# AIM-Harvard/pyradiomics

Hardware: AMD Instinct MI355X
Metric: Mvoxels/s for GLCM+GLRLM build, 512^3 vol @32 bins (higher is better)
Workload: dtype u8 levels / u32 counts / f64 out; 1 GPU; GLCM+GLRLM matrix build, 512^3 int32+uint8 volume resident in HBM, 32 grey levels, full mask, 13 angles, uniform levels; one volume per GPU (batch sharding, no collective); size=512, levels=32, dist=uniform, deferred_mode=pipeline

## Files before the change

pyradiomics_amd/csrc/kernels_sweep.h:

```cpp
#pragma once
#include "prad_runtime.h"

namespace prad {

typedef unsigned int u32;
typedef unsigned long long u64;

__global__ void __launch_bounds__(256) pack_levels_kernel(const int *__restrict__ image,
                                                          const uint8_t *__restrict__ mask, long long n, int NX,
                                                          int pitch, int padw, int Ng,
                                                          uint8_t *__restrict__ levels, int *__restrict__ flags,
                                                          int vec_ok, int shift, uint8_t *__restrict__ rowzero = nullptr) {
  const long long tid = (long long)blockIdx.x * blockDim.x + threadIdx.x;
  const long long nthreads = (long long)gridDim.x * blockDim.x;
  const bool linear = (padw == 0 && pitch == NX);
  int bad = 0;
  long long done = 0;
  if (vec_ok) {
    const long long n16 = n >> 4;
    const int upr = NX >> 4;
    const int4 *im4 = reinterpret_cast<const int4 *>(image);
    const uint4 *mk4 = reinterpret_cast<const uint4 *>(mask);
    for (long long t = tid; t < n16; t += nthreads) {
      const uint4 m = mk4[t];
// ... 682 lines not shown
    int y = r / Nx, x = r - y * Nx;
    const int pz = z - dz, py = y - dy, px = x - dx;
    if ((unsigned)pz < (unsigned)Nz && (unsigned)py < (unsigned)Ny && (unsigned)px < (unsigned)Nx) continue;
    int cnt = 0;
    while ((unsigned)z < (unsigned)Nz && (unsigned)y < (unsigned)Ny && (unsigned)x < (unsigned)Nx) {
      cnt += L[((long long)z * Ny + y) * pitch + x] != 0;
      if (cnt > 1) {
        multi[a] = 1;
        return;
      }
      z += dz; y += dy; x += dx;
    }
  }
}

__global__ void finalize_glcm_kernel(const u32 *__restrict__ acc, const u32 *__restrict__ glrlm_acc, int Ng, int Nr,
                                     int Na, int diag_from_runs, double *__restrict__ out) {
  const long long idx = (long long)blockIdx.x * blockDim.x + threadIdx.x;
  const long long total = (long long)Ng * Ng * Na;
  if (idx >= total) return;
  const int a = (int)(idx % Na);
  const long long ij = idx / Na;
  const int i = (int)(ij / Ng), j = (int)(ij - (long long)i * Ng);
  if (diag_from_runs && i == j) return;
  out[idx] = (double)acc[(size_t)a * Ng * Ng + ij];
}

__global__ void __launch_bounds__(256) finalize_glcm_diag_kernel(const u32 *__restrict__ glcm_acc, u32 *glrlm_acc, int Ng, int Nr,
                                                                 int Na, int nb1, double *__restrict__ glcm_out,
                                                                 int *__restrict__ multi, int restore_from = -1) {
  if ((int)blockIdx.x < nb1) {
    const long long idx = (long long)blockIdx.x * blockDim.x + threadIdx.x;
    const long long total = (long long)Ng * Ng * Na;
    if (idx >= total) return;
    const int a = (int)(idx % Na);
    const long long ij = idx / Na;
    const int i = (int)(ij / Ng), j = (int)(ij - (long long)i * Ng);
    if (i == j) return;
    glcm_out[idx] = (double)glcm_acc[(size_t)a * Ng * Ng + ij];
    return;
  }
  const int pair = ((int)blockIdx.x - nb1) * 4 + (int)(threadIdx.x >> 6), lane = threadIdx.x & 63;
  if (pair >= Ng * Na) return;
  const int i = pair % Ng, a = pair / Ng;
  u32 *row = glrlm_acc + ((size_t)a * Ng + i) * Nr;
  unsigned long long pairs = 0, longer = 0;
  int found = 0;
  for (int r = lane; r < Nr; r += 64) {
    const u32 v = row[r];
    pairs += (unsigned long long)r * v;
    if (r > 0) longer += v;
    found |= (r > 0 && v != 0);
  }
  const u32 *grow = glcm_acc + ((size_t)a * Ng + i) * Ng;
  for (int j = lane; j < Ng; j += 64) found |= (grow[j] != 0);
  for (int o = 32; o > 0; o >>= 1) pairs += __shfl_xor(pairs, o);
  if (lane == 0) glcm_out[((size_t)i * Ng + i) * Na + a] = (double)pairs;
  if (__ballot(found) != 0 && lane == 0) multi[a] = 1;
  if (restore_from >= 0 && a != restore_from) {
    const u32 *xrow = glrlm_acc + ((size_t)restore_from * Ng + i) * Nr;
    unsigned long long nvox = 0;
    for (int r = lane; r < Nr; r += 64) nvox += (unsigned long long)(r + 1) * xrow[r];
    for (int o = 32; o > 0; o >>= 1) {
      nvox += __shfl_xor(nvox, o);
      longer += __shfl_xor(longer, o);
    }
    if (lane == 0) row[0] = (u32)(nvox - (pairs + longer));
  }
}

__global__ void finalize_glrlm_kernel(const u32 *__restrict__ acc, const int *__restrict__ multi, int Ng, int Nr,
                                      int Na, double *__restrict__ out, const int *__restrict__ flags = nullptr,
                                      int *__restrict__ sticky = nullptr) {
  if (sticky && blockIdx.x == 0 && threadIdx.x == 0 && (flags[0] || flags[2])) sticky[0] = 1;
  const long long idx = (long long)blockIdx.x * blockDim.x + threadIdx.x;
  const long long total = (long long)Ng * Nr * Na;
  if (idx >= total) return;
  const int a = (int)(idx % Na);
  const long long gr = idx / Na;
  const int r = (int)(gr % Nr);
  out[idx] = (r == 0 && !multi[a]) ? 0.0 : (double)acc[(size_t)a * Ng * Nr + gr];
}

}
```

pyradiomics_amd/csrc/prad_api.hip:

```cpp
#include "prad_runtime.h"
#include "kernels_generic.h"
#include "kernels_pairs.h"
#include "kernels_sweep.h"
#include "kernels_sweepfw.h"
#include "kernels_sweepfw2.h"
#include "kernels_neigh.h"
#include "kernels_glszm.h"
#include "kernels_voxel.h"
#include "kernels_voxslide.h"
#include "kernels_mcc.h"
#include "kernels_voxtex.h"
#include "kernels_binning.h"

#include <algorithm>
#include <atomic>
#include <chrono>
#include <cmath>
#include <condition_variable>
#include <cstdlib>
#include <deque>
#include <limits>
#include <mutex>
#include <thread>

using namespace prad;

namespace {

const char *kVersion = "pyradiomics_amd 0.1.0 (gfx950)";

int angle_count(const int *size, const int *distances, int Nd, int Ndist, int bidirectional, int f2d) {
  long long total = 0;
  for (int k = 0; k < Ndist; k++) {
    const int dist = distances[k];
    if (dist < 1) return 0;
    long long shell_outer = 1, shell_inner = 1;
    for (int d = 0; d < Nd; d++) {
      if (d == f2d) continue;
      if (dist < size[d]) {
        shell_outer *= 2LL * dist + 1;
        shell_inner *= 2LL * dist - 1;
      } else {
        const long long reach = 2LL * (size[d] - 1) + 1;
        shell_outer *= reach;
        shell_inner *= reach;
      }
    }
    total += shell_outer - shell_inner;
  }
  if (!bidirectional) total /= 2;
  return (int)total;
}

int angle_build(const int *size, const int *distances, int Nd, int Ndist, int f2d, int Na, int *angles) {
  int maxd = 0;
  for (int k = 0; k < Ndist; k++) {
    if (distances[k] < 1) return 1;
    maxd = std::max(maxd, distances[k]);
  }
  std::vector<int> off(Nd, maxd);
  int got = 0;
  long long guard = 1;
  for (int d = 0; d < Nd; d++) guard *= (2LL * maxd + 1);
  for (long long it = 0; it < guard && got < Na; it++) {
    int norm = 0;
    bool legal = true;
    for (int d = 0; d < Nd && legal; d++) {
      const int o = off[d];
      if ((d == f2d && o != 0) || o >= size[d] || o <= -size[d]) legal = false;
      norm = std::max(norm, std::abs(o));
    }
    if (legal && norm >= 1) {
      for (int k = 0; k < Ndist; k++)
        if (distances[k] == norm) {
          std::copy(off.begin(), off.end(), angles + (size_t)got * Nd);
          got++;
          break;
        }
    }
    for (int d = Nd - 1; d >= 0; d--) {
      if (off[d] > -maxd) { off[d]--; break; }
      off[d] = maxd;
    }
  }
  return got == Na ? 0 : 1;
}

struct Call {
  Context *c;
  hipStream_t s;
  Geo g;
  VoxMode vm;
  const int32_t *image;
  const uint8_t *mask;
  const int *angles_h;
  int *angles_d;
  int Na;
  int *flags_d;
  int *flags_h;
};

int setup_call(Call &k, const int32_t *image, const uint8_t *mask, const int *size, int Nd, const int *angles,
               int Na, int Nvox, const int *voxels_dev, int kernelRadius, int force2Ddim, hipStream_t s,
               bool zero_flags = true) {
  Context &c = ctx();
  k.c = &c;
  k.s = s;
  if (!image || !mask) return fail(PRAD_E_ARG, "image/mask is NULL");
  if (!angles || Na < 1) return fail(PRAD_E_ARG, "angles is NULL or Na < 1");
  PRAD_TRY(make_geo(size, Nd, &k.g));
  if (Nvox < 1) return fail(PRAD_E_ARG, "Nvox=%d < 1", Nvox);
  k.vm.nvox = Nvox;
  k.vm.voxels = voxels_dev;
  k.vm.radius = kernelRadius;
  k.vm.f2d = force2Ddim;
  if (voxels_dev) {
    if (kernelRadius <= 0) return fail(PRAD_E_ARG, "Expecting kernelRadius > 0");
    long long b = 1;
    for (int d = 0; d < Nd; d++)
      if (d != force2Ddim) b *= std::min<long long>(2LL * kernelRadius + 1, k.g.size[d]);
    k.vm.boxmax = b;
  } else {
    if (Nvox != 1) return fail(PRAD_E_ARG, "Nvox=%d without a voxel list", Nvox);
    k.vm.boxmax = k.g.n;
  }
  k.image = image;
  k.mask = mask;
  k.angles_h = angles;
  k.Na = Na;
  {
    int *prev = nullptr;
    auto it = c.bufs.find(c.key("angles"));
    if (it != c.bufs.end()) prev = (int *)it->second.p;
    PRAD_TRY(c.get<int>("angles", (size_t)Na * Nd, &k.angles_d));
    std::vector<int> &cached = c.angle_cache();
    const bool same = prev == k.angles_d && cached.size() == (size_t)Na * Nd &&
                      std::equal(cached.begin(), cached.end(), angles);
    if (!same) {
      PRAD_HIP(hipMemcpyAsync(k.angles_d, angles, sizeof(int) * Na * Nd, hipMemcpyHostToDevice, s));
      PRAD_HIP(hipStreamSynchronize(s));
      cached.assign(angles, angles + (size_t)Na * Nd);
    }
  }
  PRAD_TRY(c.get<int>("flags", 4, &k.flags_d));
  if (zero_flags) PRAD_HIP(hipMemsetAsync(k.flags_d, 0, sizeof(int) * 4, s));
  void *fh = nullptr;
  PRAD_TRY(c.get_pinned("flags_h", sizeof(int) * 4, &fh));
  k.flags_h = (int *)fh;
  return PRAD_OK;
}

int read_flags(Call &k) {
  PRAD_HIP(hipMemcpyAsync(k.flags_h, k.flags_d, sizeof(int) * 4, hipMemcpyDeviceToHost, k.s));
  PRAD_HIP(hipStreamSynchronize(k.s));
  return PRAD_OK;
}

inline unsigned blocks_for(long long threads, int bs = 256) { return (unsigned)((threads + bs - 1) / bs); }

int check_grid(long long threads, const char *what) {
  if ((threads + 255) / 256 > 2147483647LL)
    return fail(PRAD_E_UNSUPPORTED, "%s: %lld work items exceed the launch grid; split the voxel batch", what, threads);
  return PRAD_OK;
}

int generic_glcm(Call &k, int Ng, double *out) {
  const size_t per = (size_t)Ng * Ng * k.Na;
  PRAD_HIP(hipMemsetAsync(out, 0, sizeof(double) * per * k.vm.nvox, k.s));
  const long long threads = (long long)k.vm.nvox * k.vm.boxmax;
  PRAD_TRY(check_grid(threads, "GLCM"));
  Timed t(*k.c, "generic", k.s);
  hipLaunchKernelGGL(gen_glcm_kernel, dim3(blocks_for(threads)), dim3(256), 0, k.s, k.g, k.vm, k.image, k.mask,
                     k.angles_d, k.Na, Ng, out, k.flags_d + 1);
  return check_launch("gen_glcm_kernel");
}

int generic_glrlm(Call &k, int Ng, int Nr, double *out) {
  const size_t per = (size_t)Ng * Nr * k.Na;
  PRAD_HIP(hipMemsetAsync(out, 0, sizeof(double) * per * k.vm.nvox, k.s));
  int *multi = nullptr;
  PRAD_TRY(k.c->get<int>("multi", (size_t)k.vm.nvox * k.Na, &multi));
  PRAD_HIP(hipMemsetAsync(multi, 0, sizeof(int) * k.vm.nvox * k.Na, k.s));
  const long long threads = (long long)k.vm.nvox * k.vm.boxmax * k.Na;
  PRAD_TRY(check_grid(threads, "GLRLM"));
  Timed t(*k.c, "generic", k.s);
  hipLaunchKernelGGL(gen_glrlm_kernel, dim3(blocks_for(threads)), dim3(256), 0, k.s, k.g, k.vm, k.image, k.mask,
                     k.angles_d, k.Na, Ng, Nr, out, multi, k.flags_d + 1);
  PRAD_TRY(check_launch("gen_glrlm_kernel"));
  const long long pthreads = (long long)k.vm.nvox * Ng * k.Na;
  hipLaunchKernelGGL(glrlm_prune_kernel, dim3(blocks_for(pthreads)), dim3(256), 0, k.s, out, multi, k.vm.nvox, Ng,
                     Nr, k.Na);
  return check_launch("glrlm_prune_kernel");
}

int generic_gldm(Call &k, int Ng, int alpha, double *out) {
  const size_t per = (size_t)Ng * (2 * (size_t)k.Na + 1);
  PRAD_HIP(hipMemsetAsync(out, 0, sizeof(double) * per * k.vm.nvox, k.s));
  const long long threads = (long long)k.vm.nvox * k.vm.boxmax;
  PRAD_TRY(check_grid(threads, "GLDM"));
  Timed t(*k.c, "generic", k.s);
  hipLaunchKernelGGL(gen_gldm_kernel, dim3(blocks_for(threads)), dim3(256), 0, k.s, k.g, k.vm, k.image, k.mask,
                     k.angles_d, k.Na, Ng, alpha, out, k.flags_d + 1);
  return check_launch("gen_gldm_kernel");
}

int generic_ngtdm(Call &k, int Ng, double *out) {
  Timed t(*k.c, "generic", k.s);
  if (k.vm.voxels) {
    hipLaunchKernelGGL(gen_ngtdm_voxel_kernel, dim3(blocks_for(k.vm.nvox, 64)), dim3(64), 0, k.s, k.g, k.vm,
                       k.image, k.mask, k.angles_d, k.Na, Ng, out, k.flags_d + 1);
    return check_launch("gen_ngtdm_voxel_kernel");
  }
  unsigned long long *acc = nullptr;
  const size_t nacc = (size_t)Ng * (k.Na + 1);
  PRAD_TRY(k.c->get<unsigned long long>("ngtdm_acc", nacc, &acc));
  PRAD_HIP(hipMemsetAsync(acc, 0, sizeof(unsigned long long) * nacc, k.s));
  PRAD_TRY(check_grid(k.g.n, "NGTDM"));
  hipLaunchKernelGGL(gen_ngtdm_segment_kernel, dim3(blocks_for(k.g.n)), dim3(256), 0, k.s, k.g, k.vm, k.image,
                     k.mask, k.angles_d, k.Na, Ng, acc, k.flags_d + 1);
  PRAD_TRY(check_launch("gen_ngtdm_segment_kernel"));
  hipLaunchKernelGGL(ngtdm_finalize_kernel, dim3(blocks_for(Ng, 64)), dim3(64), 0, k.s, acc, Ng, k.Na, out);
  return check_launch("ngtdm_finalize_kernel");
}

struct SweepPlan {
  bool ok = false;
  int Nz = 1, Ny = 1, Nx = 1;
  SweepSet lines;
// ... 377 lines not shown
                   int *work, int *flags_d) {
  if (pj.n16 > 0) return launch_fw2_khsp<LNG, K, HASPAD, SKIP1, true>(k, p, pj, levels16, Ng, Nr, glcm_acc, glrlm_acc, work, flags_d);
  return launch_fw2_khsp<LNG, K, HASPAD, SKIP1, false>(k, p, pj, levels16, Ng, Nr, glcm_acc, glrlm_acc, work, flags_d);
}
template <bool LNG, int K>
int launch_fw2_k(Call &k, const SweepPlan &p, const PackJob &pj, const uint8_t *levels16, int Ng, int Nr, u32 *glcm_acc, u32 *glrlm_acc,
                 int *multi, int *flags_d) {
  int *work = multi + 2 * PRAD_MAX_SWEEP + PRAD_FW_WORK_STRIDE;
  if (p.Nx != 64 * K)
    return p.skip1 ? launch_fw2_khs<LNG, K, true, true>(k, p, pj, levels16, Ng, Nr, glcm_acc, glrlm_acc, work, flags_d)
                   : launch_fw2_khs<LNG, K, true, false>(k, p, pj, levels16, Ng, Nr, glcm_acc, glrlm_acc, work, flags_d);
  return p.skip1 ? launch_fw2_khs<LNG, K, false, true>(k, p, pj, levels16, Ng, Nr, glcm_acc, glrlm_acc, work, flags_d)
                 : launch_fw2_khs<LNG, K, false, false>(k, p, pj, levels16, Ng, Nr, glcm_acc, glrlm_acc, work, flags_d);
}
int launch_fw2(Call &k, const SweepPlan &p, const PackJob &pj, const uint8_t *levels16, int Ng, int Nr, u32 *glcm_acc, u32 *glrlm_acc,
               int *multi, int *flags_d) {
  if (p.LONGfw2) return p.fwK == 4 ? launch_fw2_k<true, 4>(k, p, pj, levels16, Ng, Nr, glcm_acc, glrlm_acc, multi, flags_d)
                                 : launch_fw2_k<true, 8>(k, p, pj, levels16, Ng, Nr, glcm_acc, glrlm_acc, multi, flags_d);
  return p.fwK == 4 ? launch_fw2_k<false, 4>(k, p, pj, levels16, Ng, Nr, glcm_acc, glrlm_acc, multi, flags_d)
                    : launch_fw2_k<false, 8>(k, p, pj, levels16, Ng, Nr, glcm_acc, glrlm_acc, multi, flags_d);
}

template <bool LNG>
int launch_fw_rows(Call &k, const SweepPlan &p, const uint8_t *levels, int Ng, int Nr, u32 *glcm_acc, u32 *glrlm_acc, int *flags_d) {
  const long long nrows = (long long)p.Nz * p.Ny, groups = nrows >= 4096 ? ((nrows + 511) / 512) * 8 : (nrows + 63) / 64;
  const int wpb = p.fw_rows_threads / 64;
  const unsigned gx = (unsigned)std::max<long long>(1, std::min<long long>((groups + wpb - 1) / wpb, (long long)cu_count()));
  PRAD_HIP(hipFuncSetAttribute(reinterpret_cast<const void *>(&sweep_fw_rows_kernel<LNG>),
                               hipFuncAttributeMaxDynamicSharedMemorySize, (int)p.lds_fw_rows));
  hipLaunchKernelGGL((sweep_fw_rows_kernel<LNG>), dim3(gx), dim3(p.fw_rows_threads), p.lds_fw_rows, k.s, levels, nrows, p.Nx,
                     p.pitch, p.row_slot, Ng, Nr, p.RSfw_rows, glcm_acc, glrlm_acc, flags_d);
  return check_launch("sweep_fw_rows_kernel");
}

template <bool LNG>
int launch_fw2_rows(Call &k, const SweepPlan &p, const uint8_t *levels16, int Ng, int Nr, u32 *glcm_acc, u32 *glrlm_acc, int *flags_d) {
  const long long nrows = (long long)p.Nz * p.Ny, groups = nrows >= 4096 ? ((nrows + 511) / 512) * 8 : (nrows + 63) / 64;
  const int wpb = p.fw2r_waves;
  const unsigned gx = (unsigned)std::max<long long>(1, std::min<long long>((groups + wpb - 1) / wpb, (long long)cu_count()));
  PRAD_HIP(hipFuncSetAttribute(reinterpret_cast<const void *>(&sweep_fw2_rows_kernel<LNG>),
                               hipFuncAttributeMaxDynamicSharedMemorySize, (int)p.lds_fw2_rows));
  hipLaunchKernelGGL((sweep_fw2_rows_kernel<LNG>), dim3(gx), dim3(64 * wpb), p.lds_fw2_rows, k.s, levels16, nrows, p.Nx, p.pitch16,
                     p.row_slot, Ng, Nr, p.RS2r, p.fw2r_copies, glcm_acc, glrlm_acc, flags_d);
  return check_launch("sweep_fw2_rows_kernel");
}

template <bool G, bool R, bool LNG, bool F>
int launch_rows(Call &k, const SweepPlan &p, const uint8_t *levels, int Ng, int Nr, u32 *glcm_acc, u32 *glrlm_acc,
                int *multi) {
  const long long nrows = (long long)p.Nz * p.Ny;
  const long long groups = (nrows + 63) / 64;
  const int wpb = kRowsThreads / 64;
  const int per_cu = std::max(1, std::min(2048 / kRowsThreads, (int)(160 * 1024 / p.lds_bytes_rows)));
  const unsigned gx = (unsigned)std::max<long long>(1, std::min<long long>((groups + wpb - 1) / wpb, (long long)cu_count() * per_cu));
  PRAD_HIP(hipFuncSetAttribute(reinterpret_cast<const void *>(&sweep_rows_kernel<G, R, LNG, F>),
                               hipFuncAttributeMaxDynamicSharedMemorySize, (int)p.lds_bytes_rows));
  hipLaunchKernelGGL((sweep_rows_kernel<G, R, LNG, F>), dim3(gx), dim3(kRowsThreads), p.lds_bytes_rows, k.s, levels,
                     nrows, p.Nx, p.pitch, p.row_slot, Ng, Nr, p.RSr, glcm_acc, glrlm_acc, multi, k.flags_d);
  return check_launch("sweep_rows_kernel");
}

__global__ void __launch_bounds__(256) zero3_kernel(u32 *__restrict__ a, size_t na, u32 *__restrict__ b, size_t nb,
                                                    u32 *__restrict__ c3, size_t nc) {
  const size_t t = (size_t)blockIdx.x * blockDim.x + threadIdx.x, nt = (size_t)gridDim.x * blockDim.x;
  uint4 *a4 = reinterpret_cast<uint4 *>(a);
  for (size_t i = t; i < na / 4; i += nt) a4[i] = make_uint4(0, 0, 0, 0);
  for (size_t i = (na & ~(size_t)3) + t; i < na; i += nt) a[i] = 0;
  for (size_t i = t; i < nb; i += nt) b[i] = 0;
  for (size_t i = t; i < nc; i += nt) c3[i] = 0;
}

struct VolState {
  bool valid = false;
  SweepPlan p;
  int Ng = 0, Nr = 0, Na = 0;
  double *glcm = nullptr, *glrlm = nullptr;
  uint8_t *levels = nullptr, *rowzero = nullptr;
  uint8_t *levels16 = nullptr;
  u32 *acc = nullptr, *glcm_acc = nullptr, *glrlm_acc = nullptr;
  int *multi = nullptr;
  int *flags_d = nullptr;
  bool packed_inline = false;
  int lane = -1;
};

bool fin_side() {
  static const bool on = getenv("PRAD_FINALIZE_STREAM") != nullptr && atoi(getenv("PRAD_FINALIZE_STREAM")) != 0;
  return on;
}
int fin_wait_for_lane(hipStream_t s, int lane);

int vol_prepare(Call &k, const SweepPlan &p, int Ng, int Nr, double *glcm, double *glrlm, VolState &v) {
  Context &c = *k.c;
  if (fin_side() && c.lane >= 0) PRAD_TRY(fin_wait_for_lane(k.s, c.lane));
  v.lane = c.lane;
  v.valid = true;
  v.p = p;
  v.Ng = Ng;
  v.Nr = Nr;
  v.Na = k.Na;
  v.glcm = glcm;
  v.glrlm = glrlm;
  v.flags_d = k.flags_d;
  const long long nrows = (long long)p.Nz * p.Ny;
  v.levels = nullptr;
  if (!(p.fw2 && p.fw2_rows && p.lines.count > 0 && p.row_slot >= 0) || getenv("PRAD_FW2_KEEP8")) {
    PRAD_TRY(c.get<uint8_t>("levels", (size_t)nrows * p.pitch + 1024, &v.levels));
    v.levels += 512;
  }
  v.levels16 = nullptr;
  if (p.fw2) {
    PRAD_TRY(c.get<uint8_t>("levels16", (size_t)nrows * p.pitch16 + 4096, &v.levels16));
    v.levels16 += 2048;
  }
  const size_t nglcm = glcm ? (size_t)k.Na * Ng * Ng : 0, nglrlm = glrlm ? (size_t)k.Na * Ng * Nr : 0;
  const size_t nctl = 2 * PRAD_MAX_SWEEP + (size_t)PRAD_FW_WORK_STRIDE * (PRAD_FW_DOMAINS * PRAD_MAX_SWEEP + 1);
  PRAD_TRY(c.get<u32>("sweep_acc", nglcm + nglrlm + nctl, &v.acc));
  v.glcm_acc = v.acc;
  v.glrlm_acc = v.acc + nglcm;
  v.multi = (int *)(v.acc + nglcm + nglrlm);
  v.rowzero = nullptr;
  if (p.fw) PRAD_TRY(c.get<uint8_t>("rowzero", (size_t)nrows + 64, &v.rowzero));
  const size_t acc_w = nglcm + nglrlm + nctl, rz_w = v.rowzero ? ((size_t)nrows + 3) / 4 : 0;
  const size_t total_w = acc_w + rz_w + 4;
  const unsigned gx = (unsigned)std::max<size_t>(1, std::min<size_t>((total_w / 4 + 255) / 256, 1024));
  hipLaunchKernelGGL(zero3_kernel, dim3(gx), dim3(256), 0, k.s, v.acc, acc_w, reinterpret_cast<u32 *>(v.rowzero), rz_w,
                     reinterpret_cast<u32 *>(v.flags_d), (size_t)4);
  return check_launch("zero3_kernel");
}

bool pipeline_volume(const SweepPlan &p, bool glcm, bool glrlm) {
  if (!(p.ok && p.lines.count > 0 && glcm && glrlm)) return false;
  return (p.fw && p.fused) || (p.fw2 && !getenv("PRAD_FW2_LANES"));
}
bool pack_inline_ok(const Call &k, const VolState &v) {
  if (!(v.glcm && v.glrlm && v.p.pitch == v.p.Nx && v.p.padw == 0 && (k.g.n % 16) == 0 &&
        ((((uintptr_t)k.image) | ((uintptr_t)k.mask) | ((uintptr_t)v.levels)) & 15) == 0))
    return false;
  if (k.g.n >= (1LL << 31)) return false;
  if (v.p.fw2) return v.levels16 && v.p.pitch16 == 2 * v.p.Nx && (((uintptr_t)v.levels16) & 15) == 0;
  return v.p.fw && v.p.fused;
}

PackJob make_pack_job(const Call &k, const VolState &v, const VolState *host) {
  PackJob j;
  memset(&j, 0, sizeof(j));
  j.image = k.image;
  j.mask = k.mask;
  j.levels = v.levels;
  j.levels16 = v.p.fw2 ? v.levels16 : nullptr;
  j.rowzero = v.rowzero;
  j.flags = v.flags_d;
  j.n16 = k.g.n / 16;
  j.NX = v.p.Nx;
  j.Ng = v.Ng;
  double groups = 0, waves = 16.0;
  if (host) {
    for (int i = 0; i < host->p.fwset.count; i++) groups += (double)host->p.fwset.d[i].NM * host->p.fwset.d[i].NU / PRAD_FW_U;
    waves = 16.0 * std::max(1, host->p.fw_blocks);
  }
  const double units = (double)j.n16 / 64.0;
  const double slack = v.p.fw2 ? 1.05 : 0.92;
  j.every = (int)std::max(1.0, std::min(64.0, std::floor(slack * groups / std::max(1.0, units))));
  (void)waves;
  if (const char *e = getenv("PRAD_PACK_EVERY")) j.every = std::max(1, atoi(e));
  return j;
}

int vol_pack_standalone(Call &k, VolState &v) {
  Context &c = *k.c;
  const SweepPlan &p = v.p;
  Timed t(c, "pack", k.s);
  if (p.fw2) {
    const unsigned gx = (unsigned)std::max<long long>(1, std::min<long long>((k.g.n / 4 + 255) / 256, 8192));
    hipLaunchKernelGGL(pack_levels16_kernel, dim3(gx), dim3(256), 0, k.s, k.image, k.mask, k.g.n, p.Nx, p.pitch16, p.pitch, v.Ng,
                       v.levels16, v.levels, v.flags_d);
    return check_launch("pack_levels16_kernel");
  }
  const int vec_ok = p.vec_rows && ((((uintptr_t)k.image) | ((uintptr_t)k.mask) | ((uintptr_t)v.levels)) & 15) == 0;
  const unsigned gx = (unsigned)std::max<long long>(1, std::min<long long>((k.g.n / 16 + 255) / 256, 4096));
  const int shift = (v.glcm && v.glrlm && p.fused) ? PRAD_FUSED_SHIFT : 0;
  hipLaunchKernelGGL(pack_levels_kernel, dim3(gx), dim3(256), 0, k.s, k.image, k.mask, k.g.n, p.Nx, p.pitch, p.padw,
                     v.Ng, v.levels, v.flags_d, vec_ok, shift, v.rowzero);
  return check_launch("pack_levels_kernel");
}

template <bool G, bool R, bool F>
int launch_sweeps(Call &k, const VolState &v, const PackJob &pj) {
  const SweepPlan &p = v.p;
  if (p.lines.count > 0 && p.fw && G && R && F) {
    static const bool rows_side = getenv("PRAD_ROWS_STREAM") != nullptr;
    if (rows_side && p.row_slot >= 0) {
      static thread_local hipStream_t side = nullptr;
      static thread_local hipEvent_t e0 = nullptr, e1 = nullptr;
      if (!side) {
        int lo = 0, hi = 0;
        PRAD_HIP(hipDeviceGetStreamPriorityRange(&lo, &hi));
        PRAD_HIP(hipStreamCreateWithPriority(&side, hipStreamNonBlocking, getenv("PRAD_ROWS_STREAM_PRIO") ? atoi(getenv("PRAD_ROWS_STREAM_PRIO")) : lo));
        PRAD_HIP(hipEventCreateWithFlags(&e0, hipEventDisableTiming));
        PRAD_HIP(hipEventCreateWithFlags(&e1, hipEventDisableTiming));
      }
      PRAD_HIP(hipEventRecord(e0, k.s));
      PRAD_HIP(hipStreamWaitEvent(side, e0, 0));
      {
        Timed t(*k.c, "sweep", k.s);
        PRAD_TRY(launch_fw(k, p, pj, v.levels, v.rowzero, v.Ng, v.Nr, v.glcm_acc, v.glrlm_acc, v.multi, v.flags_d));
// ... 3 lines not shown
      if (p.RSfw_rows < v.Nr) PRAD_TRY(launch_fw_rows<true>(k2, p, v.levels, v.Ng, v.Nr, v.glcm_acc, v.glrlm_acc, v.flags_d));
      else PRAD_TRY(launch_fw_rows<false>(k2, p, v.levels, v.Ng, v.Nr, v.glcm_acc, v.glrlm_acc, v.flags_d));
      PRAD_HIP(hipEventRecord(e1, side));
      PRAD_HIP(hipStreamWaitEvent(k.s, e1, 0));
      return PRAD_OK;
    }
    {
      Timed t(*k.c, "sweep", k.s);
      PRAD_TRY(launch_fw(k, p, pj, v.levels, v.rowzero, v.Ng, v.Nr, v.glcm_acc, v.glrlm_acc, v.multi, v.flags_d));
    }
    if (p.row_slot >= 0) {
      Timed t(*k.c, "rows", k.s);
      if (p.RSfw_rows < v.Nr) PRAD_TRY(launch_fw_rows<true>(k, p, v.levels, v.Ng, v.Nr, v.glcm_acc, v.glrlm_acc, v.flags_d));
      else PRAD_TRY(launch_fw_rows<false>(k, p, v.levels, v.Ng, v.Nr, v.glcm_acc, v.glrlm_acc, v.flags_d));
    }
    return PRAD_OK;
  }
  if (p.fw2 && G && R && !F && p.lines.count > 0) {
    {
      Timed t(*k.c, "sweep", k.s);
      PRAD_TRY(launch_fw2(k, p, pj, v.levels16, v.Ng, v.Nr, v.glcm_acc, v.glrlm_acc, v.multi, v.flags_d));
    }
    if (p.row_slot >= 0) {
      Timed t(*k.c, "rows", k.s);
      if (p.fw2_rows) {
        if (p.LONGfw2r) PRAD_TRY(launch_fw2_rows<true>(k, p, v.levels16, v.Ng, v.Nr, v.glcm_acc, v.glrlm_acc, v.flags_d));
        else PRAD_TRY(launch_fw2_rows<false>(k, p, v.levels16, v.Ng, v.Nr, v.glcm_acc, v.glrlm_acc, v.flags_d));
      } else if (p.LONGr) {
        PRAD_TRY((launch_rows<G, R, true, F>(k, p, v.levels, v.Ng, v.Nr, v.glcm_acc, v.glrlm_acc, v.multi)));
      } else {
        PRAD_TRY((launch_rows<G, R, false, F>(k, p, v.levels, v.Ng, v.Nr, v.glcm_acc, v.glrlm_acc, v.multi)));
      }
    }
    return PRAD_OK;
  }
  Timed t(*k.c, "sweep", k.s);
  if (p.lines.count > 0) {
    if (R && p.LONG) PRAD_TRY((launch_lines<G, R, true, F>(k, p, v.levels, v.Ng, v.Nr, v.glcm_acc, v.glrlm_acc, v.multi)));
    else PRAD_TRY((launch_lines<G, R, false, F>(k, p, v.levels, v.Ng, v.Nr, v.glcm_acc, v.glrlm_acc, v.multi)));
  }
  if (p.row_slot >= 0) {
    if (R && p.LONGr) PRAD_TRY((launch_rows<G, R, true, F>(k, p, v.levels, v.Ng, v.Nr, v.glcm_acc, v.glrlm_acc, v.multi)));
    else PRAD_TRY((launch_rows<G, R, false, F>(k, p, v.levels, v.Ng, v.Nr, v.glcm_acc, v.glrlm_acc, v.multi)));
  }
  return PRAD_OK;
}

int vol_sweep(Call &k, const VolState &v, const PackJob &pj) {
  if (pj.n16 > 0 && !pipeline_volume(v.p, v.glcm != nullptr, v.glrlm != nullptr))
    return fail(PRAD_E_ARG, "internal: a pack job needs a fixed-window host launch");
  if (pj.n16 > 0 && (pj.levels16 != nullptr) != v.p.fw2)
    return fail(PRAD_E_ARG, "internal: the pack job's layout is not the host launch's");
  if (v.glcm && v.glrlm && v.p.fused) return launch_sweeps<true, true, true>(k, v, pj);
  if (v.glcm && v.glrlm) return launch_sweeps<true, true, false>(k, v, pj);
  if (v.glcm) return launch_sweeps<true, false, false>(k, v, pj);
  return launch_sweeps<false, true, false>(k, v, pj);
}

__global__ void latch_flags_kernel(const int *__restrict__ flags, int *__restrict__ sticky) {
  if (flags[0] || flags[2]) sticky[0] = 1;
}

__global__ void latch_any_flag_kernel(const int *__restrict__ flags, int *__restrict__ sticky) {
  if (flags[0] || flags[1] || flags[2]) sticky[0] = 1;
}
int latch_neigh(Context &c, Call &k) {
  int *sticky = nullptr;
  PRAD_TRY(c.get<int>("deferred_sticky", 16, &sticky));
  hipLaunchKernelGGL(latch_any_flag_kernel, dim3(1), dim3(1), 0, k.s, (const int *)k.flags_d, sticky);
  return check_launch("latch_any_flag_kernel");
}

int vol_finalize(Call &k, const VolState &v, int *sticky) {
  Context &c = *k.c;
  const SweepPlan &p = v.p;
  const int Ng = v.Ng, Nr = v.Nr, Na = v.Na;
  double *glcm = v.glcm, *glrlm = v.glrlm;
  bool latched = false;
  {
    Timed t(c, "finalize", k.s);
    const bool runs_diag = p.fused || p.fw2;
    if (p.fw2 && p.skip1 && p.lines.count > 0 && !(glcm && glrlm && p.row_slot >= 0))
      return fail(PRAD_E_UNSUPPORTED, "sweep plan derives runs of length 1 but the call cannot restore them");
    if (glcm && glrlm && runs_diag) {
      const int nb1 = (int)blocks_for((long long)Ng * Ng * Na), nb2 = (Ng * Na + 3) / 4;
      hipLaunchKernelGGL(finalize_glcm_diag_kernel, dim3(nb1 + nb2), dim3(256), 0, k.s, v.glcm_acc, v.glrlm_acc, Ng, Nr, Na, nb1,
                         glcm, v.multi, (p.fw2 && p.skip1 && p.lines.count > 0) ? p.row_slot : -1);
      PRAD_TRY(check_launch("finalize_glcm_diag_kernel"));
    } else if (glcm) {
      hipLaunchKernelGGL(finalize_glcm_kernel, dim3(blocks_for((long long)Ng * Ng * Na)), dim3(256), 0, k.s,
                         v.glcm_acc, v.glrlm_acc, Ng, Nr, Na, p.fused ? 1 : 0, glcm);
      PRAD_TRY(check_launch("finalize_glcm_kernel"));
    }
    if (glrlm && runs_diag) {
      if (!glcm) {
        hipLaunchKernelGGL(glcm_diag_resolve_kernel, dim3(Ng, Na), dim3(64), 0, k.s, v.glcm_acc, v.glrlm_acc, Ng, Nr, Na,
                           glcm, v.multi);
        PRAD_TRY(check_launch("glcm_diag_resolve_kernel"));
      }
      if (v.levels)
        hipLaunchKernelGGL(multi_check_kernel<uint8_t>, dim3(128, Na), dim3(256), 0, k.s, p.aset, (const uint8_t *)v.levels, p.Nz, p.Ny,
                           p.Nx, p.pitch, v.multi);
      else
        hipLaunchKernelGGL(multi_check_kernel<unsigned short>, dim3(128, Na), dim3(256), 0, k.s, p.aset,
                           reinterpret_cast<const unsigned short *>(v.levels16), p.Nz, p.Ny, p.Nx, p.pitch16 / 2, v.multi);
      PRAD_TRY(check_launch("multi_check_kernel"));
    }
    if (glrlm) {
      hipLaunchKernelGGL(finalize_glrlm_kernel, dim3(blocks_for((long long)Ng * Nr * Na)), dim3(256), 0, k.s,
                         v.glrlm_acc, v.multi, Ng, Nr, Na, glrlm, (const int *)v.flags_d, sticky);
      PRAD_TRY(check_launch("finalize_glrlm_kernel"));
      latched = sticky != nullptr;
    }
  }
  if (sticky && !latched) {
    hipLaunchKernelGGL(latch_flags_kernel, dim3(1), dim3(1), 0, k.s, v.flags_d, sticky);
    PRAD_TRY(check_launch("latch_flags_kernel"));
  }
  return PRAD_OK;
}

int sweep_glcm_glrlm(Call &k, const SweepPlan &p, int Ng, int Nr, double *glcm, double *glrlm, bool *used) {
  Context &c = *k.c;
  VolState v;
  PRAD_TRY(vol_prepare(k, p, Ng, Nr, glcm, glrlm, v));
  PRAD_TRY(vol_pack_standalone(k, v));
  PackJob pj;
  memset(&pj, 0, sizeof(pj));
  PRAD_TRY(vol_sweep(k, v, pj));
  int *sticky = nullptr;
  if (c.deferred) PRAD_TRY(c.get<int>("deferred_sticky", 16, &sticky));
  PRAD_TRY(vol_finalize(k, v, sticky));
  if (c.deferred) {
    *used = true;
    return PRAD_OK;
  }
  PRAD_TRY(read_flags(k));
  *used = (k.flags_h[0] == 0 && k.flags_h[2] == 0);
  return PRAD_OK;
}

struct PipeState {
  VolState pending;
  hipStream_t s = nullptr;
  unsigned long long seq = 0;
  hipEvent_t ev = nullptr;
  int mode = -1;
  hipStream_t fin = nullptr;
  hipEvent_t fin_in = nullptr, fin_all = nullptr, fin_done[4] = {};
  bool fin_used[4] = {};
};
PipeState &pipe_state() {
  static thread_local PipeState p;
  return p;
}
bool pipeline_mode() {
  PipeState &ps = pipe_state();
  if (ps.mode < 0) {
    const char *e = getenv("PRAD_DEFERRED_MODE");
    ps.mode = (e && strcmp(e, "lanes") == 0) ? 0 : 1;
  }
  return ps.mode == 1;
}
int pipeline_sticky(Context &c, int **sticky) { return c.get<int>("deferred_sticky", 16, sticky); }

int pipeline_retire(Context &c, hipStream_t s, const PackJob &pj) {
// ... 136 lines not shown
      RT = PRAD_PAIR_LDS_WORDS / Ng;
      ntile = (Ng + RT - 1) / RT;
    }
    const int npass = ((k.Na + AG - 1) / AG) * ntile;
    const size_t lds = sizeof(u32) * (size_t)AG * RT * Ng;
    PRAD_HIP(hipFuncSetAttribute(reinterpret_cast<const void *>(&pairs_glcm_kernel), hipFuncAttributeMaxDynamicSharedMemorySize, (int)lds));
    long long gbest = 1;
    double ebest = 0;
    for (long long gtry = std::max<long long>(1, 2LL * cus / npass); gtry <= std::max<long long>(1, (4LL * cus + npass - 1) / npass); gtry++) {
      const long long total = gtry * npass, rounds = (total + cus - 1) / cus;
      const double eff = (double)total / (double)(rounds * cus);
      if (eff > ebest + 1e-9) {
        ebest = eff;
        gbest = gtry;
      }
    }
    const unsigned gx = (unsigned)std::max<long long>(1, std::min<long long>((k.g.n / 8 + 1023) / 1024, gbest));
    hipLaunchKernelGGL(pairs_glcm_kernel, dim3(gx, (unsigned)npass), dim3(1024), lds, s, L, dims[0], dims[1], dims[2], A, AG, RT,
                       ntile, Ng, gacc, k.flags_d);
    PRAD_TRY(check_launch("pairs_glcm_kernel"));
    const long long total = (long long)Ng * Ng * k.Na;
    hipLaunchKernelGGL(finalize_glcm_kernel, dim3(blocks_for(total)), dim3(256), 0, s, gacc, (const u32 *)nullptr, Ng, 1, k.Na, 0, glcm);
    PRAD_TRY(check_launch("finalize_glcm_kernel"));
  }
  if (glrlm) {
    Timed t(c, "pairs", s);
    PRAD_HIP(hipMemsetAsync(racc, 0, sizeof(u32) * rwords, s));
    PRAD_HIP(hipMemsetAsync(counts, 0, sizeof(u32) * (size_t)Ng, s));
    PRAD_HIP(hipMemsetAsync(multi, 0, sizeof(int) * PRAD_PAIR_MAXA, s));
    const int use_lds = Ng <= 8192;
    const unsigned gc = (unsigned)std::max<long long>(1, std::min<long long>((k.g.n + 255) / 256, (long long)cus * 8));
    hipLaunchKernelGGL(pairs_level_count_kernel, dim3(gc), dim3(256), use_lds ? sizeof(u32) * (size_t)Ng : 0, s, L, k.g.n, Ng, use_lds,
                       counts, k.flags_d);
    PRAD_TRY(check_launch("pairs_level_count_kernel"));
    const unsigned gx = (unsigned)std::max<long long>(1, std::min<long long>((k.g.n + 255) / 256, std::max(1LL, 16LL * cus / k.Na)));
    hipLaunchKernelGGL(pairs_glrlm_kernel, dim3(gx, (unsigned)k.Na), dim3(256), 0, s, L, dims[0], dims[1], dims[2], A, Ng, Nr, racc, multi,
                       k.flags_d);
    PRAD_TRY(check_launch("pairs_glrlm_kernel"));
    hipLaunchKernelGGL(pairs_multi_check_kernel, dim3(gx, (unsigned)k.Na), dim3(256), 0, s, A, L, dims[0], dims[1], dims[2], multi, k.flags_d);
    PRAD_TRY(check_launch("pairs_multi_check_kernel"));
    hipLaunchKernelGGL(pairs_run1_kernel, dim3((unsigned)((Ng * k.Na + 3) / 4)), dim3(256), 0, s, racc, counts, Ng, Nr, k.Na, k.flags_d);
    PRAD_TRY(check_launch("pairs_run1_kernel"));
    const long long total = (long long)Ng * Nr * k.Na;
    hipLaunchKernelGGL(finalize_glrlm_kernel, dim3(blocks_for(total)), dim3(256), 0, s, racc, multi, Ng, Nr, k.Na, glrlm,
                       (const int *)nullptr, (int *)nullptr);
    PRAD_TRY(check_launch("finalize_glrlm_kernel"));
  }
  PRAD_TRY(read_flags(k));
  *used = k.flags_h[0] == 0;
  if (!*used) {
    PRAD_HIP(hipMemsetAsync(k.flags_d, 0, sizeof(int) * 4, s));
  }
  return PRAD_OK;
}

int texture_pairs_runs(const int32_t *image, const uint8_t *mask, const int *size, int Nd, const int *angles,
                       int Na, int Ng, int Nr, int Nvox, const int *voxels, int kernelRadius, int force2Ddim,
                       double *glcm, double *glrlm, hipStream_t s) {
  if (!glcm && !glrlm) return fail(PRAD_E_ARG, "both outputs are NULL");
  if (Ng < 1 || (glrlm && Nr < 1)) return fail(PRAD_E_ARG, "Ng/Nr must be >= 1");
  Context &c = ctx();
  PRAD_TRY(c.ensure_device());
  struct LaneGuard {
    Context &c;
    ~LaneGuard() { c.lane = -1; }
  } lane_guard{c};
  bool pipe = c.deferred && !voxels && pipeline_mode();
  if (c.deferred && !voxels && !pipe) PRAD_TRY(c.lane_begin(s, &s));
  if (pipe) c.lane = (int)(pipe_state().seq++ % (fin_side() ? 3u : 2u));
  Call k;
  PRAD_TRY(setup_call(k, image, mask, size, Nd, angles, Na, Nvox, voxels, kernelRadius, force2Ddim, s, false));
  SweepPlan p = plan_sweep(k, Ng, Nr, glcm != nullptr, glrlm != nullptr);
  if (pipe && !pipeline_volume(p, glcm != nullptr, glrlm != nullptr)) {
    const hipStream_t user = s;
    PRAD_TRY(pipeline_flush(c));
    pipe = false;
    c.lane = -1;
    PRAD_TRY(c.lane_begin(user, &s));
    if (c.lane >= 0) c.lane += fin_side() ? 3 : 2;
    PRAD_TRY(setup_call(k, image, mask, size, Nd, angles, Na, Nvox, voxels, kernelRadius, force2Ddim, s, false));
    p = plan_sweep(k, Ng, Nr, glcm != nullptr, glrlm != nullptr);
  }
  PRAD_TRY(c.begin_call(s));
  if (!p.ok) PRAD_HIP(hipMemsetAsync(k.flags_d, 0, sizeof(int) * 4, s));
  bool done = false;
  c.last_variant = !p.ok ? "none" : (p.fw2 ? "fw2" : (p.fw && glcm && glrlm ? "fw" : "lines"));
  if (pipe) {
    PRAD_TRY(pipeline_step(k, p, Ng, Nr, glcm, glrlm, &done));
    if (done) c.last_path = "sweep";
  }
  if (!done && p.ok) {
    PRAD_TRY(sweep_glcm_glrlm(k, p, Ng, Nr, glcm, glrlm, &done));
    if (done) c.last_path = "sweep";
  }
  if (!done && !c.deferred) {
    PRAD_TRY(pairs_glcm_glrlm(k, Ng, Nr, glcm, glrlm, &done));
    if (done) {
      c.last_path = "pairs";
      c.last_variant = "pairs";
    }
  }
  if (!done) {
    if (glcm) PRAD_TRY(generic_glcm(k, Ng, glcm));
    if (glrlm) PRAD_TRY(generic_glrlm(k, Ng, Nr, glrlm));
    PRAD_TRY(read_flags(k));
    c.last_path = "generic";
  }
  PRAD_TRY(c.end_call(s));
  if (c.deferred && done) return PRAD_OK;
  PRAD_HIP(hipStreamSynchronize(s));
  return k.flags_h[1] ? PRAD_INDEX_ERROR : PRAD_OK;
}

int pairs_neigh(Call &k, bool ngtdm, int Ng, int alpha, double *out, bool *used, bool box_only = false) {
  *used = false;
  Context &c = *k.c;
  if (k.vm.voxels || k.g.nd > 3 || Ng < 1 || Ng > 65535 || k.g.n >= 0x7fffffffLL || getenv("PRAD_NO_PAIRS")) return PRAD_OK;
  int dims[3] = {1, 1, 1};
  for (int d = 0; d < k.g.nd; d++) dims[3 - k.g.nd + d] = k.g.size[d];
  int rad[3] = {0, 0, 0};
  bool box = ngtdm && !getenv("PRAD_NGTDM_NO_BOX");
  long long cube = 1;
  if (box) {
    for (int a = 0; a < k.Na; a++)
      for (int d = 0; d < k.g.nd; d++) rad[3 - k.g.nd + d] = std::max(rad[3 - k.g.nd + d], std::abs(k.angles_h[a * k.g.nd + d]));
    cube = (long long)(2 * rad[0] + 1) * (2 * rad[1] + 1) * (2 * rad[2] + 1);
    box = cube - 1 == k.Na && cube <= 4096 && cube * Ng < (1LL << 40);
    if (box) {
      std::vector<char> seen((size_t)cube, 0);
      for (int a = 0; box && a < k.Na; a++) {
        long long idx = 0;
        bool zero = true;
        for (int d = 0; d < 3; d++) {
          const int o = d < 3 - k.g.nd ? 0 : k.angles_h[a * k.g.nd + (d - (3 - k.g.nd))];
          zero = zero && o == 0;
          idx = idx * (2 * rad[d] + 1) + (o + rad[d]);
        }
        if (zero || seen[(size_t)idx]) box = false;
        else seen[(size_t)idx] = 1;
      }
    }
  }
  if (box_only && !box) return PRAD_OK;
  if (!box && k.Na > PRAD_PAIR_MAXA) return PRAD_OK;
  PairAngles A;
  memset(&A, 0, sizeof(A));
  A.n = std::min(k.Na, PRAD_PAIR_MAXA);
  for (int a = 0; a < A.n; a++)
    for (int d = 0; d < k.g.nd; d++) {
      const int o = k.angles_h[a * k.g.nd + d];
      if (o < -127 || o > 127) return PRAD_OK;
      A.o[a][3 - k.g.nd + d] = (signed char)o;
    }
  const size_t nacc = (size_t)Ng * (k.Na + 1);
  if (nacc * sizeof(u64) > ((size_t)1 << 30)) return PRAD_OK;
  hipStream_t s = k.s;
  lev16 *L = nullptr;
  u32 *acc32 = nullptr;
  u64 *acc64 = nullptr;
  PRAD_TRY(c.get<lev16>("pairs_levels", (size_t)k.g.n + 8, &L));
  if (ngtdm) PRAD_TRY(c.get<u64>("pairs_ngtdm_acc", nacc, &acc64));
  else PRAD_TRY(c.get<u32>("pairs_gldm_acc", nacc, &acc32));
  PRAD_HIP(hipMemsetAsync(k.flags_d, 0, sizeof(int) * 4, s));
  const int cus = cu_count();
  {
    Timed t(c, "pack", s);
    const unsigned gx = (unsigned)std::max<long long>(1, std::min<long long>((k.g.n + 255) / 256, (long long)cus * 16));
    hipLaunchKernelGGL(pairs_pack_kernel, dim3(gx), dim3(256), 0, s, k.image, k.mask, k.g.n, Ng, L, k.flags_d);
    PRAD_TRY(check_launch("pairs_pack_kernel"));
  }
  {
    Timed t(c, "pairs", s);
    if (ngtdm) PRAD_HIP(hipMemsetAsync(acc64, 0, sizeof(u64) * nacc, s));
    else PRAD_HIP(hipMemsetAsync(acc32, 0, sizeof(u32) * nacc, s));
    const size_t budget = (size_t)PRAD_PAIR_LDS_WORDS * 4;
    int mode = 0;
    size_t lds = 0;
// ... 407 lines not shown
extern "C" {

const char *prad_version(void) { return kVersion; }
const char *prad_last_error(void) { return err_state().msg; }
const char *prad_last_path(void) { return ctx().last_path; }
const char *prad_last_variant(void) { return ctx().last_variant; }
#ifdef PRAD_FW_STAMPS
int prad_debug_fw_stamps(unsigned long long *out, int slot, int nwaves) {
  if (!out || nwaves < 1 || nwaves > 8192 || slot < 0 || slot > 1) return PRAD_E_ARG;
  PRAD_HIP(hipDeviceSynchronize());
  PRAD_HIP(hipMemcpyFromSymbol(out, HIP_SYMBOL(prad::prad_fw_stamps), sizeof(unsigned long long) * prad::FP_COUNT * (size_t)nwaves,
                               sizeof(unsigned long long) * prad::FP_COUNT * 8192 * (size_t)slot));
  return PRAD_OK;
}
#endif

int prad_device_count(void) {
  int n = 0;
  if (hipGetDeviceCount(&n) != hipSuccess) return 0;
  return n;
}

int prad_set_device(int device) {
  int n = prad_device_count();
  if (device < 0 || device >= n) return fail(PRAD_E_ARG, "device %d not in [0,%d)", device, n);
  Context &c = ctx();
  if (c.device != device) {
    if (pipe_state().pending.valid && c.device_set && hipSetDevice(c.device) == hipSuccess) {
      (void)pipeline_flush(c);
      if (pipe_state().s) (void)hipStreamSynchronize(pipe_state().s);
      (void)fin_join(nullptr, true);
    }
    pipe_state().pending.valid = false;
    pipe_state().s = nullptr;
    pipe_state().ev = nullptr;
    pipe_state().fin = nullptr;
    for (int l = 0; l < 4; l++) pipe_state().fin_used[l] = false;
    c.own_stream = nullptr;
    for (int l = 0; l < PRAD_MAX_LANES; l++) {
      if (c.lane_stream[l]) (void)hipStreamSynchronize(c.lane_stream[l]);
      c.lane_stream[l] = nullptr;
      c.lane_in[l] = nullptr;
    }
    c.event_pool.clear();
    c.events_used = 0;
  }
  c.device = device;
  c.device_set = true;
  PRAD_HIP(hipSetDevice(device));
  return PRAD_OK;
}
int prad_get_device(void) { return ctx().device; }

long long prad_workspace_bytes(void) {
  long long total = 0;
  for (const auto &kv : ctx().bufs) total += (long long)kv.second.cap;
  return total;
}
namespace {
void release_image_queues();
}
int prad_release_workspace(void) {
  Context &c = ctx();
  if (pipe_state().pending.valid) {
    (void)pipeline_flush(c);
    if (pipe_state().s) (void)hipStreamSynchronize(pipe_state().s);
    (void)fin_join(nullptr, true);
    pipe_state().pending.valid = false;
  }
  glszm_state().valid = false;
  for (auto &kv : c.bufs) {
    if (kv.second.p) (void)hipFree(kv.second.p);
    kv.second.p = nullptr;
    kv.second.cap = 0;
  }
  (void)hipDeviceSynchronize();
  for (auto &kv : c.pinned) {
    if (kv.second.p) (void)hipHostFree(kv.second.p);
    kv.second.p = nullptr;
    kv.second.cap = 0;
  }
  c.bufs.clear();
  c.pinned.clear();
  if (c.arena) (void)hipHostFree(c.arena);
  c.arena = nullptr;
  c.arena_pos = 0;
  release_image_queues();
  c.angles_cached.clear();
  StageRing &r = stage_ring();
  for (int i = 0; i < kStageRing; i++) {
    r.buf[i] = nullptr;
    r.busy[i] = false;
  }
  return PRAD_OK;
}

int prad_timing_begin(void) {
  Context &c = ctx();
  c.timing_only.clear();
  c.timing_accumulate = true;
  c.all_times.clear();
  c.all_calls.clear();
  c.events_used = 0;
  return PRAD_OK;
}
int prad_timing_begin_only(const char *kernel_family) {
  if (!kernel_family || !*kernel_family) return fail(PRAD_E_ARG, "timing: no kernel family named");
  int rc = prad_timing_begin();
  ctx().timing_only = kernel_family;
  return rc;
}
int prad_timing_count(const char *kernel_family) {
  Context &c = ctx();
  if (!kernel_family) return (int)c.all_calls.size();
  int n = 0;
  for (auto &t : c.all_times) n += t.family == kernel_family;
  return n;
}
int prad_timing_end(void) {
  Context &c = ctx();
  c.timing_only.clear();
  c.timing_accumulate = false;
  c.all_times.clear();
  c.all_calls.clear();
  return PRAD_OK;
}
int prad_timing_calls(void) { return (int)ctx().all_calls.size(); }
double prad_timing_ms(const char *family) {
  Context &c = ctx();
  double total = 0;
  if (!family) {
    for (auto &ab : c.all_calls) {
      float ms = 0;
      if (hipEventSynchronize(ab.second) != hipSuccess || hipEventElapsedTime(&ms, ab.first, ab.second) != hipSuccess) return -1.0;
      total += ms;
    }
    return total;
  }
  for (auto &t : c.all_times) {
    if (t.family != family) continue;
    float ms = 0;
    if (hipEventSynchronize(t.b) != hipSuccess || hipEventElapsedTime(&ms, t.a, t.b) != hipSuccess) return -1.0;
    total += ms;
  }
  return total;
}

int prad_set_deferred(int on) {
  Context &c = ctx();
  if (c.ensure_device() != PRAD_OK) return PRAD_E_HIP;
  if (on && !c.has("deferred_sticky")) {
    int *sticky = nullptr;
    PRAD_TRY(c.get<int>("deferred_sticky", 16, &sticky));
    PRAD_HIP(hipMemset(sticky, 0, sizeof(int) * 16));
  }
  c.deferred = on != 0;
  return PRAD_OK;
}
int prad_set_lanes(int n) {
  Context &c = ctx();
  if (n < 0 || n > PRAD_MAX_LANES) return fail(PRAD_E_ARG, "lanes=%d outside [0, %d]", n, PRAD_MAX_LANES);
  PRAD_TRY(c.lanes_sync());
  c.lanes = n;
  c.lane_seq = 0;
  return PRAD_OK;
}
// ... 673 lines not shown
```

Baseline: 287,200 Mvoxels/s.

## Fuse GLCM/GLRLM finalize, multi-check and accumulator zeroing into one tail kernel

Adds a single finalize_tail_kernel per angle that computes the GLCM diagonal from run counts, restores length-1 runs, performs the multi-run check, writes both f64 outputs and zeroes the accumulators, control words and rowzero for the next call. Host-side state tracks whether the accumulators are already clean, so the next vol_prepare can skip the full zero3 clear or only clear the leftover slice. This removes several small kernel launches and a separate memset pass per volume. The cost is more complex cross-call state that must be invalidated correctly, and a fallback multi-check scan inside the fused kernel.

```diff
diff --git a/pyradiomics_amd/csrc/kernels_sweep.h b/pyradiomics_amd/csrc/kernels_sweep.h
--- a/pyradiomics_amd/csrc/kernels_sweep.h
+++ b/pyradiomics_amd/csrc/kernels_sweep.h
@@ -788,4 +788,99 @@
   out[idx] = (r == 0 && !multi[a]) ? 0.0 : (double)acc[(size_t)a * Ng * Nr + gr];
 }
 
-}
+template <typename T>
+__global__ void __launch_bounds__(1024) finalize_tail_kernel(u32 *glcm_acc, u32 *glrlm_acc, int *ctl, int nctl, int Ng, int Nr, int Na,
+                                                             double *__restrict__ glcm_out, double *__restrict__ glrlm_out,
+                                                             int restore_from, AngleSet A, const T *__restrict__ L, int Nz, int Ny,
+                                                             int Nx, int pitch, u32 *rowzero, unsigned rz_w, int *flags,
+                                                             int *__restrict__ sticky, int zero, int clear_flags) {
+  __shared__ unsigned long long s_pairs[256], s_longer[256], s_nvox[256];
+  const int a = blockIdx.y, S = gridDim.x, s = blockIdx.x;
+  const int tid = threadIdx.x, lane = tid & 63, wave = tid >> 6, nw = blockDim.x >> 6;
+  const int i0 = (int)((long long)Ng * s / S), i1 = (int)((long long)Ng * (s + 1) / S);
+  u32 *gacc = glcm_acc + (size_t)a * Ng * Ng;
+  u32 *racc = glrlm_acc + (size_t)a * Ng * Nr;
+  const bool restore = restore_from >= 0 && a != restore_from;
+  if (s == 0 && a == 0 && tid == 0) {
+    if (sticky && (flags[0] || flags[2])) sticky[0] = 1;
+    if (clear_flags) flags[0] = flags[1] = flags[2] = flags[3] = 0;
+  }
+  int found = (tid == 0 && ctl[a] != 0);
+  for (int i = wave; i < Ng; i += nw) {
+    const u32 *row = racc + (size_t)i * Nr;
+    unsigned long long pairs = 0, longer = 0, nvox = 0;
+    for (int r = lane; r < Nr; r += 64) {
+      const u32 v = row[r];
+      pairs += (unsigned long long)r * v;
+      if (r > 0) longer += v;
+    }
+    found |= (longer != 0);
+    const u32 *grow = gacc + (size_t)i * Ng;
+    for (int j = lane; j < Ng; j += 64) found |= (grow[j] != 0);
+    if (restore && i >= i0 && i < i1) {
+      const u32 *xrow = glrlm_acc + ((size_t)restore_from * Ng + i) * Nr;
+      for (int r = lane; r < Nr; r += 64) nvox += (unsigned long long)(r + 1) * xrow[r];
+    }
+    for (int o = 32; o > 0; o >>= 1) {
+      pairs += __shfl_xor(pairs, o);
+      longer += __shfl_xor(longer, o);
+      nvox += __shfl_xor(nvox, o);
+    }
+    if (lane == 0) {
+      s_pairs[i] = pairs;
+      s_longer[i] = longer;
+      s_nvox[i] = nvox;
+    }
+  }
+  int multi = __syncthreads_or(found);
+  if (!multi) {
+    const int dz = A.off[a][0], dy = A.off[a][1], dx = A.off[a][2];
+    if ((dz < 0 ? -dz : dz) < Nz && (dy < 0 ? -dy : dy) < Ny && (dx < 0 ? -dx : dx) < Nx) {
+      const long long n = (long long)Nz * Ny * Nx, plane = (long long)Ny * Nx;
+      for (long long base = 0; base < n && !multi; base += (long long)blockDim.x * 8) {
+        int hit = 0;
+        for (int q = 0; q < 8 && !hit; q++) {
+          const long long i = base + (long long)q * blockDim.x + tid;
+          if (i >= n) break;
+          int z = (int)(i / plane);
+          const int rem = (int)(i - (long long)z * plane);
+          int y = rem / Nx, x = rem - y * Nx;
+          const int pz = z - dz, py = y - dy, px = x - dx;
+          if ((unsigned)pz < (unsigned)Nz && (unsigned)py < (unsigned)Ny && (unsigned)px < (unsigned)Nx) continue;
+          int cnt = 0;
+          while ((unsigned)z < (unsigned)Nz && (unsigned)y < (unsigned)Ny && (unsigned)x < (unsigned)Nx) {
+            cnt += L[((long long)z * Ny + y) * pitch + x] != 0;
+            if (cnt > 1) {
+              hit = 1;
+              break;
+            }
+            z += dz; y += dy; x += dx;
+          }
+        }
+        multi = __syncthreads_or(hit);
+      }
+    }
+  }
+  for (int idx = i0 * Ng + tid; idx < i1 * Ng; idx += blockDim.x) {
+    const int i = idx / Ng, j = idx - i * Ng;
+    const u32 v = gacc[idx];
+    glcm_out[(size_t)idx * Na + a] = i == j ? (double)s_pairs[i] : (double)v;
+    if (zero) gacc[idx] = 0;
+  }
+  const bool zero_runs = zero && !(restore_from >= 0 && a == restore_from);
+  for (long long idx = (long long)i0 * Nr + tid; idx < (long long)i1 * Nr; idx += blockDim.x) {
+    const int i = (int)(idx / Nr), r = (int)(idx - (long long)i * Nr);
+    u32 v = racc[idx];
+    if (r == 0 && restore) v = (u32)(s_nvox[i] - (s_pairs[i] + s_longer[i]));
+    glrlm_out[(size_t)idx * Na + a] = (r == 0 && !multi) ? 0.0 : (double)v;
+    if (zero_runs) racc[idx] = 0;
+  }
+  if (zero) {
+    for (int w = tid; w < nctl; w += blockDim.x)
+      if (w % Na == a) ctl[w] = 0;
+    const unsigned w0 = (unsigned)((unsigned long long)rz_w * a / Na), w1 = (unsigned)((unsigned long long)rz_w * (a + 1) / Na);
+    for (unsigned w = w0 + tid; w < w1; w += blockDim.x) rowzero[w] = 0;
+  }
+}
+
+}
diff --git a/pyradiomics_amd/csrc/prad_api.hip b/pyradiomics_amd/csrc/prad_api.hip
--- a/pyradiomics_amd/csrc/prad_api.hip
+++ b/pyradiomics_amd/csrc/prad_api.hip
@@ -99,6 +99,8 @@
   int *flags_d;
   int *flags_h;
 };
+
+void tail_mark_dirty(Context &c);
 
 int setup_call(Call &k, const int32_t *image, const uint8_t *mask, const int *size, int Nd, const int *angles,
                int Na, int Nvox, const int *voxels_dev, int kernelRadius, int force2Ddim, hipStream_t s,
@@ -143,7 +145,10 @@
     }
   }
   PRAD_TRY(c.get<int>("flags", 4, &k.flags_d));
-  if (zero_flags) PRAD_HIP(hipMemsetAsync(k.flags_d, 0, sizeof(int) * 4, s));
+  if (zero_flags) {
+    PRAD_HIP(hipMemsetAsync(k.flags_d, 0, sizeof(int) * 4, s));
+    tail_mark_dirty(c);
+  }
   void *fh = nullptr;
   PRAD_TRY(c.get_pinned("flags_h", sizeof(int) * 4, &fh));
   k.flags_h = (int *)fh;
@@ -687,7 +692,33 @@
   int *flags_d = nullptr;
   bool packed_inline = false;
   int lane = -1;
+  size_t acc_w = 0, rz_w = 0;
+  struct TailClean *tail = nullptr;
 };
+
+struct TailClean {
+  bool clean = false;
+  hipStream_t s = nullptr;
+  u32 *acc = nullptr, *rowzero = nullptr;
+  size_t acc_w = 0, rz_w = 0;
+  int *flags = nullptr;
+  bool flags_clean = false;
+  u32 *left = nullptr;
+  size_t left_w = 0;
+};
+std::map<std::string, TailClean> &tail_states() {
+  static thread_local std::map<std::string, TailClean> m;
+  return m;
+}
+void tail_mark_dirty(Context &c) {
+  auto it = tail_states().find(c.key("sweep_acc"));
+  if (it != tail_states().end()) it->second.clean = false;
+}
+bool fin_side();
+bool tail_merge_on() {
+  const char *e = getenv("PRAD_OLD_FINALIZE");
+  return !(e && atoi(e) != 0) && !fin_side();
+}
 
 bool fin_side() {
   static const bool on = getenv("PRAD_FINALIZE_STREAM") != nullptr && atoi(getenv("PRAD_FINALIZE_STREAM")) != 0;
@@ -727,6 +758,21 @@
   v.rowzero = nullptr;
   if (p.fw) PRAD_TRY(c.get<uint8_t>("rowzero", (size_t)nrows + 64, &v.rowzero));
   const size_t acc_w = nglcm + nglrlm + nctl, rz_w = v.rowzero ? ((size_t)nrows + 3) / 4 : 0;
+  v.acc_w = acc_w;
+  v.rz_w = rz_w;
+  TailClean &tc = tail_states()[c.key("sweep_acc")];
+  v.tail = &tc;
+  const TailClean was = tc;
+  tc.clean = false;
+  if (tail_merge_on() && was.clean && was.s == k.s && was.acc == v.acc && was.acc_w >= acc_w && was.flags == v.flags_d &&
+      (!v.rowzero || (was.rowzero == reinterpret_cast<u32 *>(v.rowzero) && was.rz_w >= rz_w))) {
+    if (was.left_w == 0 && was.flags_clean) return PRAD_OK;
+    const size_t fw = was.flags_clean ? 0 : 4;
+    const unsigned gl = (unsigned)std::max<size_t>(1, std::min<size_t>((was.left_w + 255) / 256, 1024));
+    hipLaunchKernelGGL(zero3_kernel, dim3(gl), dim3(256), 0, k.s, (u32 *)nullptr, (size_t)0, was.left, was.left_w,
+                       reinterpret_cast<u32 *>(v.flags_d), fw);
+    return check_launch("zero3_kernel");
+  }
   const size_t total_w = acc_w + rz_w + 4;
   const unsigned gx = (unsigned)std::max<size_t>(1, std::min<size_t>((total_w / 4 + 255) / 256, 1024));
   hipLaunchKernelGGL(zero3_kernel, dim3(gx), dim3(256), 0, k.s, v.acc, acc_w, reinterpret_cast<u32 *>(v.rowzero), rz_w,
@@ -896,6 +942,38 @@
     const bool runs_diag = p.fused || p.fw2;
     if (p.fw2 && p.skip1 && p.lines.count > 0 && !(glcm && glrlm && p.row_slot >= 0))
       return fail(PRAD_E_UNSUPPORTED, "sweep plan derives runs of length 1 but the call cannot restore them");
+    if (glcm && glrlm && runs_diag && tail_merge_on()) {
+      const long long per_angle = (long long)Ng * ((long long)Nr + Ng);
+      int S = per_angle <= 4096 ? 1 : (int)std::min<long long>(std::min(16, Ng), (per_angle + 2047) / 2048);
+      if (const char *e = getenv("PRAD_TAIL_SLICES")) S = std::max(1, std::min(std::min(64, Ng), atoi(e)));
+      const int zero = S == 1 ? 1 : 0, clear_flags = (zero && sticky) ? 1 : 0;
+      const int restore_from = (p.fw2 && p.skip1 && p.lines.count > 0) ? p.row_slot : -1;
+      const int nctl = (int)(v.acc_w - (size_t)Na * Ng * Ng - (size_t)Na * Ng * Nr);
+      if (v.levels)
+        hipLaunchKernelGGL(finalize_tail_kernel<uint8_t>, dim3(S, Na), dim3(1024), 0, k.s, v.glcm_acc, v.glrlm_acc, v.multi, nctl, Ng, Nr,
+                           Na, glcm, glrlm, restore_from, p.aset, (const uint8_t *)v.levels, p.Nz, p.Ny, p.Nx, p.pitch,
+                           reinterpret_cast<u32 *>(v.rowzero), (unsigned)v.rz_w, v.flags_d, sticky, zero, clear_flags);
+      else
+        hipLaunchKernelGGL(finalize_tail_kernel<unsigned short>, dim3(S, Na), dim3(1024), 0, k.s, v.glcm_acc, v.glrlm_acc, v.multi, nctl,
+                           Ng, Nr, Na, glcm, glrlm, restore_from, p.aset, reinterpret_cast<const unsigned short *>(v.levels16), p.Nz,
+                           p.Ny, p.Nx, p.pitch16 / 2, reinterpret_cast<u32 *>(v.rowzero), (unsigned)v.rz_w, v.flags_d, sticky, zero,
+                           clear_flags);
+      PRAD_TRY(check_launch("finalize_tail_kernel"));
+      if (zero && v.tail) {
+        TailClean &tc = *v.tail;
+        tc.clean = true;
+        tc.s = k.s;
+        tc.acc = v.acc;
+        tc.acc_w = v.acc_w;
+        tc.rowzero = reinterpret_cast<u32 *>(v.rowzero);
+        tc.rz_w = v.rz_w;
+        tc.flags = v.flags_d;
+        tc.flags_clean = clear_flags != 0;
+        tc.left = restore_from >= 0 ? v.glrlm_acc + (size_t)restore_from * Ng * Nr : nullptr;
+        tc.left_w = restore_from >= 0 ? (size_t)Ng * Nr : 0;
+      }
+      return PRAD_OK;
+    }
     if (glcm && glrlm && runs_diag) {
       const int nb1 = (int)blocks_for((long long)Ng * Ng * Na), nb2 = (Ng * Na + 3) / 4;
       hipLaunchKernelGGL(finalize_glcm_diag_kernel, dim3(nb1 + nb2), dim3(256), 0, k.s, v.glcm_acc, v.glrlm_acc, Ng, Nr, Na, nb1,
@@ -1198,7 +1276,10 @@
     p = plan_sweep(k, Ng, Nr, glcm != nullptr, glrlm != nullptr);
   }
   PRAD_TRY(c.begin_call(s));
-  if (!p.ok) PRAD_HIP(hipMemsetAsync(k.flags_d, 0, sizeof(int) * 4, s));
+  if (!p.ok) {
+    PRAD_HIP(hipMemsetAsync(k.flags_d, 0, sizeof(int) * 4, s));
+    tail_mark_dirty(c);
+  }
   bool done = false;
   c.last_variant = !p.ok ? "none" : (p.fw2 ? "fw2" : (p.fw && glcm && glrlm ? "fw" : "lines"));
   if (pipe) {
@@ -1209,6 +1290,7 @@
     PRAD_TRY(sweep_glcm_glrlm(k, p, Ng, Nr, glcm, glrlm, &done));
     if (done) c.last_path = "sweep";
   }
+  if (!done) tail_mark_dirty(c);
   if (!done && !c.deferred) {
     PRAD_TRY(pairs_glcm_glrlm(k, Ng, Nr, glcm, glrlm, &done));
     if (done) {
@@ -1782,6 +1864,7 @@
   }
   c.bufs.clear();
   c.pinned.clear();
+  tail_states().clear();
   if (c.arena) (void)hipHostFree(c.arena);
   c.arena = nullptr;
   c.arena_pos = 0;
```

Measured after the change: 283,600 Mvoxels/s. 1.3% lower.
